# mozack/vdjer

Hardware: AMD Instinct MI355X
Metric: M paired-reads/sec (k-mer build + contig score), IgH 50bp PE (higher is better)
Workload: dtype u8/u64 (2-bit packed bases, integer counts)

## Files before the change

vdjer_amd/csrc/vdjx_kmer.hip:

```cpp
#include "vdjx_common.h"
#include "vdjx_scan.h"
#include "vdjx_part.h"

#include <algorithm>
#include <numeric>
#include <type_traits>
#include <string.h>
#include <stdlib.h>

#define HIST_THREADS 512
#define HIST_BLOCKS 512u
#define LOCAL_SLOTS 2048u
#define K3_SUB_TUPLES g_sub_tuples
__device__ u32 g_sub_tuples = 262144u;
#define NONE32 0xFFFFFFFFu
#define INST_MASK 0x7FFFFFFFu

struct RecView {
	u64 bhi, blo, nm, lq;
};

__device__ inline RecView load_rec(const u64* __restrict__ bases, const u64* __restrict__ nmask,
                                   const u64* __restrict__ lowq, size_t r) {
	RecView v;
// ... 296 lines not shown
                                                    u32 shift, u32 sub_bits, u32* __restrict__ fine_cnt) {
	__shared__ u32 h[PART_MAXB];
	const u32 nbk = 1u << sub_bits;
	for (u32 i = threadIdx.x; i < nbk; i += 512) h[i] = 0;
	__syncthreads();
	size_t t0, t1;
	const u32 seg = part_slice(seg_start, seg_shift, slices, t0, t1);
	for (size_t t = t0 + threadIdx.x; t < t1; t += 512) {
		const TUP x = TUP::load(&in[t]);
		atomicAdd(&h[(u32) (vdjx_bucket_mix(x.lo, x.hi()) >> shift) & (nbk - 1)], 1u);
	}
	__syncthreads();
	for (u32 i = threadIdx.x; i < nbk; i += 512) if (h[i]) atomicAdd(&fine_cnt[((size_t) seg << sub_bits) | i], h[i]);
}

#ifndef RD_THREADS
#define RD_THREADS 768
#define RD_UNR 4
#define RD_WAVES 6
#endif
#define RD_SLOTS 2048u
#define RD_SLOT_BITS 11
#define RD_PQ 4096u
#define RD_LI 512u
#define RD_LROWS 128u
#define RD_MAXLOW 11u
#define ST_CAND 1u
#define ST_MULTI 2u
#define ST_QOK 4u
#define ST_QOK_R 8u
#define ST_ID_SHIFT 8
#define ST_NOID 0xFFFFFFu

struct SurvOutG { u64* lo; u64* hi; u32* gcnt; u64* gfirst; u32* n; u32 cap; u32* n_real; };
#define GC_SHADOW 0x80000000u
#define GC_MASK 0x7FFFFFFFu

__device__ inline bool reads_equal(const u64* __restrict__ bases, const u64* __restrict__ nmask, int rl, u64 a, u64 b) {
	if (rl <= VDJX_SHORT_READ_LEN) {
		const ulonglong2 x = ((const ulonglong2*) bases)[a];
// ... 44 lines not shown
	if (threadIdx.x < 33) cls_cnt[threadIdx.x] = 0;
	__syncthreads();
	for (u32 b = threadIdx.x; b < NB; b += 1024) {
		const u32 n = bucket_start[b + 1] - bucket_start[b];
		atomicAdd(&cls_cnt[n ? 32u - (u32) __builtin_clz(n) : 0u], 1u);
	}
	__syncthreads();
	if (threadIdx.x == 0) { u32 at = 0; for (int cl = 32; cl >= 0; cl--) { cls_at[cl] = at; at += cls_cnt[cl]; } }
	__syncthreads();
	for (u32 b = threadIdx.x; b < NB; b += 1024) {
		const u32 n = bucket_start[b + 1] - bucket_start[b];
		order[atomicAdd(&cls_at[n ? 32u - (u32) __builtin_clz(n) : 0u], 1u)] = b;
	}
}

template <typename TUP, bool SYM = false>
__global__ __launch_bounds__(RD_THREADS, sizeof(TUP) == 16 ? RD_WAVES : RD_WAVES / 2) void k_gated_reduce(const TUP* __restrict__ tup, const u32* __restrict__ bucket_start,
                                                             const u64* __restrict__ bases, const u64* __restrict__ nmask,
                                                             vdjx_qrows quals, int rl, int ob, int k, u64 rec_base,
                                                             u32 mf, u32 cmin, u32 mqq, u32 tlow, SurvOutG so,
                                                             u64* __restrict__ g_distinct, u32* __restrict__ g_err, u32 dbg_in,
                                                             const u32* __restrict__ order) {
#ifdef VDJX_ABLATE
	const u32 dbg = dbg_in;
#else
	const u32 dbg = dbg_in == 9u ? 9u : 0u;
#endif
	typedef typename TUP::hi_t THI;
	__shared__ u64 s_klo[RD_SLOTS];
	__shared__ THI s_khi[RD_SLOTS];
	__shared__ u64 s_first[RD_SLOTS];
	__shared__ u32 s_cnt[RD_SLOTS], s_state[RD_SLOTS];
	__shared__ u32 pq[RD_PQ];
	__shared__ u64 low_inst[RD_LI];
	__shared__ u32 low_n[RD_LROWS];
	__shared__ unsigned short low_slot[RD_LROWS];
	__shared__ u32 s_over, s_ndist, s_nlow, s_npq, s_nsurv, s_base, s_nreal;
	const THI EMPTY = (THI) ~(THI) 0;
	const u32 b = order ? order[blockIdx.x] : blockIdx.x;
	const u32 base = bucket_start[b];
	const u32 n = bucket_start[b + 1] - base;
	const u32 tid = threadIdx.x;
	if (n == 0) return;
	const TUP* T = tup + base;
	const u32 om = (1u << ob) - 1u;
	const u32 per_low = tlow > 1 ? (tlow - 1 < RD_MAXLOW ? tlow - 1 : RD_MAXLOW) : 1;
	const u32 lrows = RD_LI / per_low < RD_LROWS ? RD_LI / per_low : RD_LROWS;
	u32 S = 1;
	while ((u64) S * K3_SUB_TUPLES < n) S <<= 1;
	u32 ndist_total = 0;
	bool verify = S > 1;
	for (;;) {
		if (tid == 0) { s_over = 0; s_ndist = 0; }
		__syncthreads();
		for (u32 s = 0; s < S; s++) {
			for (u32 i = tid; i < RD_SLOTS; i += RD_THREADS) { s_khi[i] = EMPTY; s_cnt[i] = 0; s_first[i] = NONE64; s_state[i] = 0; }
			if (tid == 0) { s_nlow = 0; s_npq = (n >> (32 - RD_SLOT_BITS) || dbg == 9) ? RD_PQ + 1 : 0; s_nsurv = 0; s_nreal = 0; }
			__syncthreads();
			for (u32 t0 = 0; t0 < n; t0 += RD_UNR * RD_THREADS) {
				TUP r_t[RD_UNR];
#pragma unroll
				for (int j = 0; j < RD_UNR; j++) {
					const u32 t = t0 + j * RD_THREADS + tid;
					if (t < n) r_t[j] = TUP::load(&T[t]);
				}
#pragma unroll
				for (int j = 0; j < RD_UNR; j++) {
					const u32 t = t0 + j * RD_THREADS + tid;
					int slot = -1;
					if (t < n) {
						const u32 h = rd_hash(r_t[j].lo, r_t[j].hi());
						if (!(S > 1 && ((h >> 12) & (S - 1)) != s)) {
							slot = lds_insert<THI, RD_SLOTS>(s_klo, s_khi, r_t[j].lo, (THI) r_t[j].hi(), h);
							if (slot < 0) s_over = 1;
						}
					}
					const bool live = slot >= 0 && !verify;
					const u64 inst = r_t[j].inst();
					const u32 c0 = rd_count_min(s_cnt, s_first, (u32) (live ? slot : 0), inst, live);
					bool list = false;
					if (live) {
						u32 st = vdjx_peek(&s_state[slot]);
// ... 2 lines not shown
							if (f != NONE64 && (f >> ob) != (inst >> ob)) {
								const u32 o1 = (u32) inst & om, o0 = (u32) f & om;
								const u32 d = o1 > o0 ? o1 - o0 : o0 - o1;
								if (d && d < (u32) k && !vdjx_kmer_has_period(r_t[j].hi(), r_t[j].lo, k, d)) { atomicOr(&s_state[slot], ST_MULTI); st |= ST_MULTI; }
							}
						}
						list = !((st & ST_MULTI) && c0 + 1 >= tlow);
					}
					const u32 qi = vdjx_wave_inc(&s_npq, list);
					if (list && qi < RD_PQ) pq[qi] = (t << RD_SLOT_BITS) | (u32) slot;
				}
			}
			__syncthreads();
			if (s_over || verify) { if (s_over) break; continue; }
			if (dbg == 1) return;
			for (u32 i = tid; i < RD_SLOTS; i += RD_THREADS) {
				if (s_khi[i] == EMPTY) continue;
				atomicAdd(&s_ndist, SYM ? 2u : 1u);
				const u32 c = s_cnt[i];
				if (c >= cmin) s_state[i] = (s_state[i] & ST_MULTI) | ST_CAND | ((c < tlow ? atomicAdd(&s_nlow, 1u) : ST_NOID) << ST_ID_SHIFT);
			}
			__syncthreads();
			const u32 nlow = s_nlow;
			const bool listed = s_npq <= RD_PQ;
			const u32 nscan = listed ? s_npq : n;
			for (u32 l0 = 0; l0 == 0 || l0 < nlow; l0 += lrows) {
				for (u32 i = tid; i < RD_LROWS; i += RD_THREADS) low_n[i] = 0;
				__syncthreads();
				for (u32 e = tid; e < nscan; e += RD_THREADS) {
					u32 slot, t;
					TUP x;
					if (listed) {
						slot = pq[e] & (RD_SLOTS - 1); t = pq[e] >> RD_SLOT_BITS;
						if (!(vdjx_peek(&s_state[slot]) & ST_CAND)) continue;
						x = TUP::load(&T[t]);
					} else {
						x = TUP::load(&T[e]);
						const u32 h = rd_hash(x.lo, x.hi());
						if (S > 1 && ((h >> 12) & (S - 1)) != s) continue;
						const int sl = lds_lookup<THI, RD_SLOTS>(s_klo, s_khi, x.lo, (THI) x.hi(), h);
						if (sl < 0) continue;
						slot = (u32) sl;
					}
					const u32 st = vdjx_peek(&s_state[slot]);
					if (!(st & ST_CAND)) continue;
					const u64 inst = x.inst(), fi = s_first[slot];
					const u32 lid = st >> ST_ID_SHIFT;
					if (lid != ST_NOID && lid >= l0 && lid < l0 + lrows) {
						const u32 pos = atomicAdd(&low_n[lid - l0], 1u);
						if (pos < per_low) low_inst[(lid - l0) * per_low + pos] = inst;
						low_slot[lid - l0] = (unsigned short) slot;
					}
					if (l0 == 0 && !(st & ST_MULTI) && (inst >> ob) != (fi >> ob)) {
						const u32 o1 = (u32) inst & om, o0 = (u32) fi & om;
						const u32 d = o1 > o0 ? o1 - o0 : o0 - o1;
						if ((d && d < (u32) k && !vdjx_kmer_has_period(x.hi(), x.lo, k, d))
						    || !reads_equal(bases, nmask, rl, (inst >> ob) - rec_base, (fi >> ob) - rec_base)) atomicOr(&s_state[slot], ST_MULTI);
					}
				}
				__syncthreads();
				if (dbg == 4) return;
				const u32 rows = nlow - l0 < lrows ? nlow - l0 : lrows;
				const u32 lane = tid & 63u;
				for (u32 r = tid >> 6; r < (nlow ? rows : 0u); r += RD_THREADS / 64) {
					const u32 slot = low_slot[r], cnt = low_n[r];
					const u64 fi = s_first[slot];
					u32 qv[RD_MAXLOW];
#pragma unroll
					for (u32 i = 0; i < RD_MAXLOW; i++) {
						qv[i] = 33u;
						if (i < cnt && i < per_low) {
							const u64 inst = low_inst[r * per_low + i];
							const uint8_t* q = quals.row((inst >> ob) - rec_base) + (inst == fi ? 0u : (u32) inst & om);
							if (lane < (u32) k) qv[i] = q[lane];
						}
					}
					u32 sum = 0;
#pragma unroll
					for (u32 i = 0; i < RD_MAXLOW; i++) sum += (u32) (uint8_t) (qv[i] - 33u);
					const bool lowq = lane < (u32) k && sum < mqq;
					if (!__ballot(lowq) && lane == 0) atomicOr(&s_state[slot], ST_QOK);
					if (SYM) {
						u64 fr = NONE64;
#pragma unroll
						for (u32 i = 0; i < RD_MAXLOW; i++)
							if (i < cnt && i < per_low) { const u64 m = vdjx_inst_mirror(low_inst[r * per_low + i], ob, rl, k); fr = m < fr ? m : fr; }
#pragma unroll
						for (u32 i = 0; i < RD_MAXLOW; i++) {
							qv[i] = 33u;
							if (i < cnt && i < per_low) {
								const u64 inst = vdjx_inst_mirror(low_inst[r * per_low + i], ob, rl, k);
								const uint8_t* q = quals.row((inst >> ob) - rec_base) + (inst == fr ? 0u : (u32) inst & om);
								if (lane < (u32) k) qv[i] = q[lane];
							}
						}
						u32 sum_r = 0;
#pragma unroll
						for (u32 i = 0; i < RD_MAXLOW; i++) sum_r += (u32) (uint8_t) (qv[i] - 33u);
						const bool lowq_r = lane < (u32) k && sum_r < mqq;
						if (!__ballot(lowq_r) && lane == 0) atomicOr(&s_state[slot], ST_QOK_R);
					}
				}
				__syncthreads();
			}
			if (dbg == 5) return;
			for (u32 i = tid; i < RD_SLOTS; i += RD_THREADS) {
				const u32 st = s_state[i];
				bool keep = false, keep_r = false;
				if (st & ST_CAND) {
					const u32 craw = s_cnt[i];
					const u32 c = craw > 32765u ? 32765u : craw;
					keep = c >= mf && (st & ST_MULTI) && (craw >= tlow || (st & ST_QOK));
					if (SYM) keep_r = c >= mf && (st & ST_MULTI) && (craw >= tlow || (st & ST_QOK_R));
				}
				if (SYM) {
					s_state[i] = (keep || keep_r) ? (atomicAdd(&s_nsurv, 2u) << 2) | (u32) keep | ((u32) keep_r << 1) : NONE32;
					if (keep || keep_r) atomicAdd(&s_nreal, (u32) keep + (u32) keep_r);
				} else s_state[i] = keep ? atomicAdd(&s_nsurv, 1u) : NONE32;
			}
			__syncthreads();
			if (tid == 0) { s_base = s_nsurv ? atomicAdd(so.n, s_nsurv) : 0; if (SYM && s_nreal) atomicAdd(so.n_real, s_nreal); }
			__syncthreads();
			for (u32 i = tid; i < RD_SLOTS; i += RD_THREADS) {
				if (s_state[i] == NONE32) continue;
				u32 pos = s_base + (SYM ? s_state[i] >> 2 : s_state[i]);
				const u32 cgo = s_cnt[i] > 32765u ? 32765u : s_cnt[i];
				if (pos < so.cap) {
					so.lo[pos] = s_klo[i];
					so.hi[pos] = (u64) s_khi[i];
					so.gcnt[pos] = cgo | (SYM && !(s_state[i] & 1u) ? GC_SHADOW : 0u);
					so.gfirst[pos] = s_first[i];
				}
				if (SYM) {
					pos += 1u;
					if (pos < so.cap) {
						u64 rh, rlo;
						vdjx_kmer_rc((u64) s_khi[i], s_klo[i], k, rh, rlo);
						so.lo[pos] = rlo;
// ... 27 lines not shown
static_assert(sizeof(PartialS) == sizeof(Partial), "vdjx_shard_record_bytes(0) is one number");
#define PS_H_BITS 26
#define PS_MAX_SPLIT (1u << (PS_H_BITS - 12))
__device__ inline u64 ps_hi(const PartialS& p) { return p.hic & 0xFFFFFFFFFFFFull; }
__device__ inline u32 ps_cg(const PartialS& p) { const u32 c = (u32) (p.hic >> 48); return (c & 0x7FFFu) | ((c & 0x8000u) ? PART_FLAG : 0u); }
__device__ inline u64 ps_fg(const PartialS& p) { return p.fgh & INST_MASK64; }
__device__ inline u32 ps_h(const PartialS& p) { return (u32) (p.fgh >> INST_BITS); }
#define NEED_SEQ 1u
#define NEED_Q 2u
#define PID_MASK 0x3FFFFFFFu
#define REPLY_KQ 52
#define REPLY_BYTES 408

#define LG_THREADS 768
#define LG_UNR 4
#define LG_FLAG 0x80000000u
#define LG_NOLIST 0x7FFFFFFFu
template <typename TUP, bool SYM = false>
__global__ __launch_bounds__(LG_THREADS, sizeof(TUP) == 16 ? 6 : 3) void k_gated_local(const TUP* __restrict__ tup, const u32* __restrict__ bucket_start,
                                                            const u64* __restrict__ bases, const u64* __restrict__ nmask, u64 rec_base, int k, int rl, int ob,
                                                            u32 tlow, Partial* __restrict__ sparse_g, u32* __restrict__ sparse_ref,
                                                            u32* __restrict__ nd_g, u64* __restrict__ low_inst, u32* __restrict__ g_err,
                                                            const u32* __restrict__ order) {
	typedef typename TUP::hi_t THI;
	const size_t obase = (size_t) bucket_start[order ? order[blockIdx.x] : blockIdx.x];
	__shared__ u64 s_klo[LOCAL_SLOTS];
	__shared__ THI s_khi[LOCAL_SLOTS];
	__shared__ u64 s_mg[LOCAL_SLOTS];
	__shared__ u32 s_cg[LOCAL_SLOTS], s_st[LOCAL_SLOTS];
	__shared__ u32 pq[RD_PQ];
	__shared__ u32 s_ng, s_nlow, s_over, s_npq;
	static_assert(LOCAL_SLOTS == (1u << RD_SLOT_BITS), "list entries carry the slot in RD_SLOT_BITS bits");
	const THI EMPTY = (THI) ~(THI) 0;
	const u32 b = order ? order[blockIdx.x] : blockIdx.x;
	const u32 base = bucket_start[b];
	const u32 n = bucket_start[b + 1] - base;
	const u32 tid = threadIdx.x;
	const u32 om = (1u << ob) - 1u;
	if (n == 0) { if (tid == 0) nd_g[b] = 0; return; }
	const TUP* T = tup + base;
	u32 S = 1;
	while ((u64) S * K3_SUB_TUPLES < n) S <<= 1;
	for (;;) {
		if (tid == 0) { s_ng = 0; s_nlow = 0; s_over = 0; }
		for (u32 s = 0; s < S; s++) {
			for (u32 i = tid; i < LOCAL_SLOTS; i += LG_THREADS) { s_khi[i] = EMPTY; s_cg[i] = 0; s_mg[i] = NONE64; s_st[i] = 0; }
			if (tid == 0) s_npq = n >> (32 - RD_SLOT_BITS) ? RD_PQ + 1 : 0;
			__syncthreads();
			for (u32 t0 = 0; t0 < n; t0 += LG_UNR * LG_THREADS) {
				TUP r_t[LG_UNR];
#pragma unroll
				for (int j = 0; j < LG_UNR; j++) {
					const u32 t = t0 + j * LG_THREADS + tid;
					if (t < n) r_t[j] = TUP::load(&T[t]);
				}
#pragma unroll
				for (int j = 0; j < LG_UNR; j++) {
					const u32 t = t0 + j * LG_THREADS + tid;
					int slot = -1;
					if (t < n) {
						const u32 h = rd_hash(r_t[j].lo, r_t[j].hi());
						if (!(S > 1 && ((h >> 12) & (S - 1)) != s)) {
// ... 6 lines not shown
					const u32 c0 = rd_count_min(s_cg, s_mg, (u32) (live ? slot : 0), inst, live);
					bool list = false;
					if (live) {
						u32 st = vdjx_peek(&s_st[slot]);
						if (!(st & LG_FLAG)) {
							const u64 f = vdjx_peek(&s_mg[slot]);
							if (f != NONE64 && (f >> ob) != (inst >> ob)) {
								const u32 o1 = (u32) inst & om, o0 = (u32) f & om;
								const u32 d = o1 > o0 ? o1 - o0 : o0 - o1;
								if (d && d < (u32) k && !vdjx_kmer_has_period(r_t[j].hi(), r_t[j].lo, k, d)) { atomicOr(&s_st[slot], LG_FLAG); st |= LG_FLAG; }
							}
						}
						list = !((st & LG_FLAG) && c0 + 1 >= tlow);
					}
					const u32 qi = vdjx_wave_inc(&s_npq, list);
					if (list && qi < RD_PQ) pq[qi] = (t << RD_SLOT_BITS) | (u32) slot;
				}
			}
			__syncthreads();
			if (s_over) break;
			for (u32 i = tid; i < LOCAL_SLOTS; i += LG_THREADS) {
				const u32 cg = s_cg[i];
				s_st[i] = (s_st[i] & LG_FLAG) | ((cg && cg < tlow) ? atomicAdd(&s_nlow, cg) : LG_NOLIST);
			}
			__syncthreads();
			const bool listed = s_npq <= RD_PQ;
			const u32 nscan = listed ? s_npq : n;
			for (u32 e = tid; e < nscan; e += LG_THREADS) {
				u32 slot;
				TUP x;
				if (listed) {
					slot = pq[e] & (LOCAL_SLOTS - 1);
					const u32 st0 = vdjx_peek(&s_st[slot]);
					if ((st0 & LG_NOLIST) == LG_NOLIST && (st0 & LG_FLAG)) continue;
					x = TUP::load(&T[pq[e] >> RD_SLOT_BITS]);
				} else {
					x = TUP::load(&T[e]);
					const u32 h = rd_hash(x.lo, x.hi());
					if (S > 1 && ((h >> 12) & (S - 1)) != s) continue;
					const int sl = lds_lookup<THI, LOCAL_SLOTS>(s_klo, s_khi, x.lo, (THI) x.hi(), h);
					if (sl < 0) continue;
					slot = (u32) sl;
				}
				const u32 st = vdjx_peek(&s_st[slot]);
				const u32 loff = st & LG_NOLIST;
				const u64 inst = x.inst();
				u32 cg = vdjx_peek(&s_cg[slot]);
				if (loff != LG_NOLIST) {
					cg &= 0xFFFFu;
					low_inst[base + loff + (atomicAdd(&s_cg[slot], 0x10000u) >> 16)] = inst;
// ... 1188 lines not shown

inline u32 ceil_log2_u64(u64 x) { u32 b = 0; while ((1ull << b) < x) b++; return b; }

static bool sync_debug() { static const bool on = vdjx_env_set("VDJX_SYNC_DEBUG"); return on; }
static void dbg_sync(vdjx_ctx* c, const char* what) {
	if (!sync_debug()) return;
	const hipError_t e = hipStreamSynchronize(c->stream);
	fprintf(stderr, "[vdjx] %s: %s\n", what, hipGetErrorString(e));
}

struct GatedHist { u32 HB = 0, NBH = 0, N = 0; u32* hstart = nullptr; bool sym = false; };
static bool build_sym(const vdjx_pool* pool, int k) {
	return pool->sym && pool->W == 2 && (k & 1) && pool->n_records % 2 == 0;
}
static bool sym_walk_wanted() { static const bool on = !vdjx_env_set("VDJX_NO_SYM_WALK"); return on; }
static size_t gated_bucket_default() { static const size_t v = (size_t) vdjx_env_num("VDJX_GATED_BUCKET", 3072, 1, 1ll << 32); return v; }
template <typename A>
int stage_gated_hist(vdjx_ctx* c, A& db, const vdjx_pool* pool, int k, size_t per_bucket, u64 geometry_instances, GatedHist* gh, bool sym = false) {
	hipStream_t st = c->stream;
	const size_t R = sym ? pool->n_records / 2 : pool->n_records;
	const int P = pool->rl - k + 1;
	const u64 NI = geometry_instances ? geometry_instances : (u64) R * (u64) P;
	const size_t per = per_bucket ? per_bucket : gated_bucket_default();
	const u32 hb_max = pool->W > 2 ? 14u : 15u;
	u32 HB = ceil_log2_u64((NI + per - 1) / per);
	HB = std::max(8u, std::min(hb_max, HB));
	const u32 NBH = 1u << HB;
#ifdef VDJX_ABLATE
	static const u32 hist_dbg = (u32) vdjx_env_num("VDJX_HIST_DBG", 0, 0, 4);
#else
	constexpr u32 hist_dbg = 0;
#endif
	u32 nblk = (u32) std::min<size_t>(HIST_BLOCKS, (R + 4095) / 4096);
	if (nblk == 0) nblk = 1;
	size_t rpb = (R + nblk - 1) / nblk;
	u32 *hcnt, *hstart;
	HIP_TRY(db.alloc(&hcnt, NBH));
	HIP_TRY(db.alloc(&hstart, NBH + 1));
// ... 12 lines not shown
	dbg_sync(c, "k_gated_hist");
	vdjx_scan_one(st, hcnt, NBH, hstart);
	HIP_TRY(hipMemcpyAsync(c->h_pin, hstart + NBH, 4, hipMemcpyDeviceToHost, st));
	HIP_TRY(hipStreamSynchronize(st));
	HIP_TRY(hipGetLastError());
#ifdef VDJX_ABLATE
	if (hist_dbg) return VDJX_ESTATE;
#endif
	const u32 N = *(const u32*) c->h_pin;
	c->stats["gated_instances"] = sym ? 2ull * N : N;
	gh->HB = HB; gh->NBH = NBH; gh->N = N; gh->hstart = hstart; gh->sym = sym;
	return VDJX_OK;
}

template <typename TUP, typename A>
int stage_gated_cut(vdjx_ctx* c, A& db, const vdjx_pool* pool, u64 rec_base, int k, size_t per_bucket, u64 geometry_instances, const GatedHist& gh, GTuples<TUP>* out) {
	hipStream_t st = c->stream;
	const bool sym = gh.sym;
	const size_t R = sym ? pool->n_records / 2 : pool->n_records;
	const int P = pool->rl - k + 1;
	const size_t per = per_bucket ? per_bucket : gated_bucket_default();
	const u32 hb_max = pool->W > 2 ? 14u : 15u;
	const bool lng = pool->W > 2;
	const u32 HB = gh.HB, NBH = gh.NBH, N = gh.N;
	u32* hstart = gh.hstart;
	size_t rpb;
	out->N = N;
	const u64 Ng = geometry_instances ? geometry_instances : (u64) N;
	static const size_t refine = (size_t) vdjx_env_num("VDJX_REFINE_TUPLES", 4096, 1, 1ll << 32);
	u32 T = 8;
	while (T < HB && ((u64) per << T) < Ng) T++;
	u32 extra = 0;
	const size_t refine_at = per_bucket ? std::max<size_t>(per_bucket, refine / 2) : refine;
	if (T == HB && HB == hb_max && Ng / NBH > refine_at) {
		extra = 1;
		while (extra < 5 && (Ng >> extra) / NBH > refine_at) extra++;
	}
	const u32 Tt = T + extra;
	const u32 NBt = 1u << Tt;
	HIP_TRY(db.alloc(&out->t, (size_t) N + 1));
	constexpr u32 stage_tuples = PARTR_STAGE_BYTES / (u32) sizeof(TUP);
	constexpr u32 lds_partr = PARTR_STAGE_BYTES + stage_tuples * 4;
	u32 cbits = Tt, fbits = 0;
	if (Tt > 10) { cbits = extra ? Tt - 10 : 8; fbits = Tt - cbits; }
// ... 29 lines not shown
		vdjx_scan_one(st, fine_cnt, NBt, tstart);
	} else {
		hipLaunchKernelGGL(k_pick_u32, dim3((NBt + 1 + 255) / 256), dim3(256), 0, st, hstart, 1u << (HB - Tt), NBt + 1, tstart);
	}
	if (fbits) {
		u32* gcur2;
		HIP_TRY(db.alloc(&gcur2, NBt));
		vdjx_prof_scope ps(c, "k_part_tuples");
		HIP_TRY(part_launch(st, k_part<TUP, TupBucket<TUP>, part_segs>, NBc * slices, PART_LDS_BYTES, tstart, NBt, 0u, gcur2, out->t,
		                    l1, part_segs{hstart, HB - cbits, slices, fbits}, TupBucket<TUP>{64 - Tt, (1u << fbits) - 1u}));
	}
	return VDJX_OK;
}

template <typename TUP, typename A>
int stage_gated_partition(vdjx_ctx* c, A& db, const vdjx_pool* pool, u64 rec_base, int k, size_t per_bucket, u64 geometry_instances, GTuples<TUP>* out, bool sym = false) {
	GatedHist gh;
	int rc = stage_gated_hist(c, db, pool, k, per_bucket, geometry_instances, &gh, sym);
	if (rc) return rc;
	return stage_gated_cut<TUP>(c, db, pool, rec_base, k, per_bucket, geometry_instances, gh, out);
}

static int set_sub_tuples(vdjx_ctx* c) {
	static const u32 sub = (u32) vdjx_env_num("VDJX_SUB_TUPLES", 262144, 1, 0xFFFFFFFFll);
	if (c->sub_tuples_set != sub) {
		HIP_TRY(hipMemcpyToSymbolAsync(HIP_SYMBOL(g_sub_tuples), &sub, 4, 0, hipMemcpyHostToDevice, c->stream));
		c->sub_tuples_set = sub;
	}
	return VDJX_OK;
}
template <typename TUP, typename A>
int bucket_order(vdjx_ctx* c, A& db, const GTuples<TUP>& t, u32** order) {
	*order = nullptr;
	if (t.NB < 1024) return VDJX_OK;
	HIP_TRY(db.alloc(order, t.NB));
// ... 14 lines not shown
	const u32 cap = (sym ? t.N : t.N / 2) + 16;
	u32 *g_err, *n_surv;
	u64* g_distinct;
	HIP_TRY(db.alloc(&sv->lo, cap)); HIP_TRY(db.alloc(&sv->hi, cap)); HIP_TRY(db.alloc(&sv->gcnt, cap)); HIP_TRY(db.alloc(&sv->gfirst, cap));
	HIP_TRY(db.alloc(&g_distinct, 64 * 16 + 2));
	g_err = (u32*) (g_distinct + 64 * 16);
	n_surv = g_err + 1;
	u32* n_real = g_err + 2;
	HIP_TRY(hipMemsetAsync(g_distinct, 0, (64 * 16 + 2) * 8, st));
	SurvOutG so{sv->lo, sv->hi, sv->gcnt, sv->gfirst, n_surv, cap, n_real};
	static const u32 rd_dbg = (u32) vdjx_env_num("VDJX_RD_DBG", 0, 0, 9);
	if (t.N) {
		vdjx_prof_scope ps(c, "k_gated_reduce");
		u32* order;
		if ((rc = bucket_order(c, db, t, &order))) return rc;
		if (sym) hipLaunchKernelGGL((k_gated_reduce<TUP, true>), dim3(t.NB), dim3(RD_THREADS), 0, st, t.t, t.bucket_start, pv.bases, pv.nmask, pv.quals, pv.rl, pv.ob, k, rec_base,
		                            mfu, cmin, mqq, tlow, so, g_distinct, g_err, rd_dbg, (const u32*) order);
		else hipLaunchKernelGGL(k_gated_reduce<TUP>, dim3(t.NB), dim3(RD_THREADS), 0, st, t.t, t.bucket_start, pv.bases, pv.nmask, pv.quals, pv.rl, pv.ob, k, rec_base,
		                        mfu, cmin, mqq, tlow, so, g_distinct, g_err, rd_dbg, (const u32*) order);
	}
	u64* spread = (u64*) c->h_pin;
	u32* tail = (u32*) (spread + 64 * 16);
	static_assert((64 * 16 + 2) * 8 == VDJX_HPIN_SYNC_BYTES, "h_pin layout (vdjx_common.h)");
	HIP_TRY(hipMemcpyAsync(spread, g_distinct, VDJX_HPIN_SYNC_BYTES, hipMemcpyDeviceToHost, st));
	HIP_TRY(hipStreamSynchronize(st));
	HIP_TRY(hipGetLastError());
	const u32 ns = tail[1], err = tail[0];
	if (err) { vdjx_set_error("k_gated_reduce: %u buckets could not be split to fit LDS", err); return VDJX_EHIP; }
	if (ns > cap) { vdjx_set_error("survivor capacity logic failed (%u > %u)", ns, cap); return VDJX_EHIP; }
	sv->ndist = 0;
// ... 380 lines not shown
	HIP_TRY(hipStreamSynchronize(st));
	HIP_TRY(hipGetLastError());
	n_roots = *(const u32*) c->h_pin;
	g->n_roots = n_roots;
	vdjx_prof_collect(c, false);
	return VDJX_OK;
}

template <typename TUP>
int kmer_build_impl2(vdjx_ctx* c, const vdjx_pool* pool, int k, int mf, int mq, vdjx_graph* g) {
	const int P = pool->rl - k + 1;
	vdjx_work db(c);
	GTuples<TUP> t;
	const bool sym = build_sym(pool, k);
	c->stats["kmer_build_sym"] = sym ? 1 : 0;
	int rc = stage_gated_partition<TUP>(c, db, pool, 0, k, 0, 0, &t, sym);
	if (rc) return rc;
	PoolView pv{pool->d_bases, pool->d_nmask, vdjx_qrows{pool->d_quals, pool->d_quals2, pool->q_split, pool->qstride}, pool->rl, pool->ob};
	SurvivorsG sv;
	rc = stage_gated_reduce<TUP>(c, db, t, pv, 0, k, mf, mq, &sv, sym);
	if (rc) return rc;
	vdjx_ri_open_gate(c);
	dbg_sync(c, "gated_reduce");
	g->pre_nodes = (size_t) sv.ndist;
	RecountOut ro{};
	if (sv.n) {
		HIP_TRY(db.alloc(&sv.ucnt, sv.n)); HIP_TRY(db.alloc(&sv.ufirst, sv.n));
		HIP_TRY(db.alloc(&ro.in_first, (size_t) sv.n * 4)); HIP_TRY(db.alloc(&ro.in_from, (size_t) sv.n * 4));
		HIP_TRY(db.alloc(&ro.edge_first, (size_t) sv.n * 4)); HIP_TRY(db.alloc(&ro.edge_to, (size_t) sv.n * 4));
		ro.ucnt = sv.ucnt; ro.ufirst = sv.ufirst;
		for (int attempt = 0; attempt < 2; attempt++) {
// ... 136 lines not shown
static u64 shard_geometry_bound(const vdjx_shard* s) {
	const int P = s->pool->rl - s->k + 1;
	return std::max<u64>(1, s->rec_stride * (u64) P / 4);
}

template <typename TUP>
static int shard_local_impl(vdjx_shard* s) {
	vdjx_ctx* c = s->c;
	hipStream_t st = c->stream;
	PersistAlloc db(c);
	const u64 rec_base = s->rec_base();
	GTuples<TUP> t;
	int rc = VDJX_OK;
	if (s->have_hist && s->gh.sym != s->sym) s->have_hist = false;
	const size_t per_b = 0;
	if (!s->have_hist) rc = stage_gated_hist(c, db, s->pool, s->k, per_b, shard_geometry_bound(s) / (s->sym ? 2 : 1), &s->gh, s->sym);
	if (rc) return rc;
	s->have_hist = true;
	const size_t cap = (size_t) s->gh.N + 1;
	const size_t nb_max = ((size_t) 1 << 20) + 16 * (size_t) s->nranks + 2;
	Partial* sparse;
	u32 *g_err, *sparse_ref;
	HIP_TRY(db.alloc(&s->low_inst, cap));
	HIP_TRY(db.alloc(&s->dense_ref, cap));
	HIP_TRY(db.alloc(&s->nd, nb_max));
	HIP_TRY(db.alloc(&s->dstart, nb_max + 1));
	HIP_TRY(db.alloc(&g_err, 1));
	u32* keep_starts;
	HIP_TRY(db.alloc(&keep_starts, nb_max + 1));
	s->fill_mark = db.mark();
	HIP_TRY(db.alloc(&sparse, cap));
	HIP_TRY(db.alloc(&sparse_ref, cap));
	const vdjx_arena::mark_t tuple_mark = db.mark();
	rc = stage_gated_cut<TUP>(c, db, s->pool, rec_base, s->k, per_b, (s->agreed ? s->agreed : shard_geometry_bound(s)) / (s->sym ? 2 : 1), s->gh, &t);
	if (rc) return rc;
	if (t.NB < (u32) s->nranks) { vdjx_set_error("vdjx_shard_local: fewer buckets (%u) than ranks", t.NB); return VDJX_ELIMIT; }
	s->NBo = t.NB / (u32) s->nranks;
	if (s->NBo * (u32) s->nranks != t.NB) s->NBo = (s->NBo + 1 + 15) & ~15u;
	s->NBf = s->NBo * (u32) s->nranks;
	if ((size_t) s->NBf + 1 > nb_max) { vdjx_set_error("vdjx_shard_local: %u buckets", s->NBf); return VDJX_ELIMIT; }
	HIP_TRY(hipMemsetAsync(g_err, 0, 4, st));
	if (s->NBf > t.NB) HIP_TRY(hipMemsetAsync(s->nd + t.NB, 0, (size_t) (s->NBf - t.NB) * 4, st));
	if ((rc = set_sub_tuples(c))) return rc;
	{
		vdjx_prof_scope ps(c, "k_gated_local");
		u32* order;
		if ((rc = bucket_order(c, db, t, &order))) return rc;
		if (s->sym) hipLaunchKernelGGL((k_gated_local<TUP, true>), dim3(t.NB), dim3(LG_THREADS), 0, st, t.t, t.bucket_start, s->pool->d_bases, s->pool->d_nmask, rec_base,
		                               s->k, s->pool->rl, s->pool->ob, s->tlow, sparse, sparse_ref, s->nd, s->low_inst, g_err, (const u32*) order);
// ... 54 lines not shown
	if (s->sparse) {
		PersistAlloc db(s->c);
		db.release_to(s->fill_mark);
		s->sparse = nullptr; s->sparse_ref = nullptr; s->tuple_bucket_start = nullptr;
	}
	return VDJX_OK;
}

extern "C" int vdjx_shard_count(vdjx_shard* s, uint64_t* gated_instances) {
	if (!s || !gated_instances) { vdjx_set_error("vdjx_shard_count: NULL argument"); return VDJX_EINVAL; }
	if (s->phase != 0) { vdjx_set_error("vdjx_shard_count: call it before vdjx_shard_local"); return VDJX_ESTATE; }
	HIP_TRY(hipSetDevice(s->c->device));
	vdjx_clear_errors();
	if (!s->have_hist) {
		PersistAlloc db(s->c);
		const int rc = stage_gated_hist(s->c, db, s->pool, s->k, 0, shard_geometry_bound(s) / (s->sym_capable ? 2 : 1), &s->gh, s->sym_capable);
		if (rc) return rc;
		s->have_hist = true;
	}
	*gated_instances = (u64) s->gh.N * (s->gh.sym ? 2 : 1);
	return VDJX_OK;
}
extern "C" int vdjx_shard_symmetric(const vdjx_shard* s) { return s && s->sym_capable ? 1 : 0; }
extern "C" int vdjx_shard_geometry2(vdjx_shard* s, uint64_t agreed_instances, int all_symmetric) {
	if (!s) { vdjx_set_error("vdjx_shard_geometry2: NULL argument"); return VDJX_EINVAL; }
	if (all_symmetric && !s->sym_capable) { vdjx_set_error("vdjx_shard_geometry2: this rank's pool is not made of couples"); return VDJX_EINVAL; }
	const int rc = vdjx_shard_geometry(s, agreed_instances);
	if (rc) return rc;
	s->sym = all_symmetric != 0;
	s->c->stats["kmer_build_sym"] = s->sym ? 1 : 0;
	return VDJX_OK;
// ... 433 lines not shown
```

Baseline: 918.8.

## Template gated-reduce geometry; prefetch first tuple batch; hoist read-compare loads

Geometry constants for the gated reduce kernel (threads, slot bits, pq size, low rows, bucket size) become a template traits struct, with a narrower variant available for 16-byte tuples. The default stays wide, and bucket and refine sizes are now derived from that geometry. The first batch of tuples is loaded before the hash table clear so global load latency overlaps the LDS init. The read-equality loads are issued before the low-row atomics, and the symmetric mirror-quality pass is merged into the forward loop. The extra registers for hoisted loads and merged SYM arrays could lower occupancy.

Result: no change. 919.7 (median of 2 runs) (+0.1%).

```diff
diff --git a/vdjer_amd/csrc/vdjx_kmer.hip b/vdjer_amd/csrc/vdjx_kmer.hip
--- a/vdjer_amd/csrc/vdjx_kmer.hip
+++ b/vdjer_amd/csrc/vdjx_kmer.hip
@@ -334,16 +334,13 @@
 	for (u32 i = threadIdx.x; i < nbk; i += 512) if (h[i]) atomicAdd(&fine_cnt[((size_t) seg << sub_bits) | i], h[i]);
 }
 
-#ifndef RD_THREADS
-#define RD_THREADS 768
-#define RD_UNR 4
-#define RD_WAVES 6
+struct RdWide   { static constexpr u32 THREADS = 768, UNR = 4, WAVES = 6, SLOT_BITS = 11, PQ = 4096, LI = 512, LROWS = 128, BUCKET = 3072; };
+struct RdNarrow { static constexpr u32 THREADS = 384, UNR = 4, WAVES = 6, SLOT_BITS = 10, PQ = 2048, LI = 256, LROWS = 64, BUCKET = 1536; };
+#ifndef VDJX_RD_GEOM16
+#define VDJX_RD_GEOM16 RdWide
 #endif
-#define RD_SLOTS 2048u
-#define RD_SLOT_BITS 11
-#define RD_PQ 4096u
-#define RD_LI 512u
-#define RD_LROWS 128u
+template <typename TUP> struct RdGeomOf { typedef RdWide type; };
+template <> struct RdGeomOf<Tup16> { typedef VDJX_RD_GEOM16 type; };
 #define RD_MAXLOW 11u
 #define ST_CAND 1u
 #define ST_MULTI 2u
@@ -418,8 +415,10 @@
 	}
 }
 
-template <typename TUP, bool SYM = false>
-__global__ __launch_bounds__(RD_THREADS, sizeof(TUP) == 16 ? RD_WAVES : RD_WAVES / 2) void k_gated_reduce(const TUP* __restrict__ tup, const u32* __restrict__ bucket_start,
+__device__ inline u32 rd_again(u32 x) { asm volatile("" : "+v"(x)); return x; }
+
+template <typename TUP, bool SYM = false, typename G = typename RdGeomOf<TUP>::type>
+__global__ __launch_bounds__(G::THREADS, sizeof(TUP) == 16 ? G::WAVES : G::WAVES / 2) void k_gated_reduce(const TUP* __restrict__ tup, const u32* __restrict__ bucket_start,
                                                              const u64* __restrict__ bases, const u64* __restrict__ nmask,
                                                              vdjx_qrows quals, int rl, int ob, int k, u64 rec_base,
                                                              u32 mf, u32 cmin, u32 mqq, u32 tlow, SurvOutG so,
@@ -431,6 +430,9 @@
 	const u32 dbg = dbg_in == 9u ? 9u : 0u;
 #endif
 	typedef typename TUP::hi_t THI;
+	constexpr u32 RD_THREADS = G::THREADS, RD_UNR = G::UNR, RD_SLOT_BITS = G::SLOT_BITS, RD_SLOTS = 1u << G::SLOT_BITS, RD_PQ = G::PQ, RD_LI = G::LI, RD_LROWS = G::LROWS;
+	static_assert(RD_SLOT_BITS <= 16, "low_slot is 16 bits wide");
+	static_assert(RD_LI >= RD_MAXLOW, "a round holds at least one row of the longest kind");
 	__shared__ u64 s_klo[RD_SLOTS];
 	__shared__ THI s_khi[RD_SLOTS];
 	__shared__ u64 s_first[RD_SLOTS];
@@ -458,18 +460,26 @@
 		if (tid == 0) { s_over = 0; s_ndist = 0; }
 		__syncthreads();
 		for (u32 s = 0; s < S; s++) {
-			for (u32 i = tid; i < RD_SLOTS; i += RD_THREADS) { s_khi[i] = EMPTY; s_cnt[i] = 0; s_first[i] = NONE64; s_state[i] = 0; }
-			if (tid == 0) { s_nlow = 0; s_npq = (n >> (32 - RD_SLOT_BITS) || dbg == 9) ? RD_PQ + 1 : 0; s_nsurv = 0; s_nreal = 0; }
+			TUP r_t[RD_UNR];
+			const u32 tid0 = rd_again(tid);
+#pragma unroll
+			for (u32 j = 0; j < RD_UNR; j++) {
+				const u32 t = j * RD_THREADS + tid0;
+				if (t < n) r_t[j] = TUP::load(&T[t]);
+			}
+			for (u32 i = rd_again(tid); i < RD_SLOTS; i += RD_THREADS) { s_khi[i] = EMPTY; s_cnt[i] = 0; s_first[i] = NONE64; s_state[i] = 0; }
+			if (tid == 0) { s_nlow = 0; s_npq = (rd_again(n) >> (32 - RD_SLOT_BITS) || dbg == 9) ? RD_PQ + 1 : 0; s_nsurv = 0; s_nreal = 0; }
 			__syncthreads();
 			for (u32 t0 = 0; t0 < n; t0 += RD_UNR * RD_THREADS) {
-				TUP r_t[RD_UNR];
+				if (t0) {
 #pragma unroll
-				for (int j = 0; j < RD_UNR; j++) {
-					const u32 t = t0 + j * RD_THREADS + tid;
-					if (t < n) r_t[j] = TUP::load(&T[t]);
+					for (u32 j = 0; j < RD_UNR; j++) {
+						const u32 t = t0 + j * RD_THREADS + tid;
+						if (t < n) r_t[j] = TUP::load(&T[t]);
+					}
 				}
 #pragma unroll
-				for (int j = 0; j < RD_UNR; j++) {
+				for (u32 j = 0; j < RD_UNR; j++) {
 					const u32 t = t0 + j * RD_THREADS + tid;
 					int slot = -1;
 					if (t < n) {
@@ -502,7 +512,7 @@
 			__syncthreads();
 			if (s_over || verify) { if (s_over) break; continue; }
 			if (dbg == 1) return;
-			for (u32 i = tid; i < RD_SLOTS; i += RD_THREADS) {
+			for (u32 i = rd_again(tid); i < RD_SLOTS; i += RD_THREADS) {
 				if (s_khi[i] == EMPTY) continue;
 				atomicAdd(&s_ndist, SYM ? 2u : 1u);
 				const u32 c = s_cnt[i];
@@ -513,15 +523,16 @@
 			const bool listed = s_npq <= RD_PQ;
 			const u32 nscan = listed ? s_npq : n;
 			for (u32 l0 = 0; l0 == 0 || l0 < nlow; l0 += lrows) {
-				for (u32 i = tid; i < RD_LROWS; i += RD_THREADS) low_n[i] = 0;
+				for (u32 i = rd_again(tid); i < RD_LROWS; i += RD_THREADS) low_n[i] = 0;
 				__syncthreads();
-				for (u32 e = tid; e < nscan; e += RD_THREADS) {
-					u32 slot, t;
+				for (u32 e = rd_again(tid); e < nscan; e += RD_THREADS) {
+					u32 slot = 0;
 					TUP x;
 					if (listed) {
-						slot = pq[e] & (RD_SLOTS - 1); t = pq[e] >> RD_SLOT_BITS;
+						const u32 ent = pq[e];
+						slot = ent & (RD_SLOTS - 1);
 						if (!(vdjx_peek(&s_state[slot]) & ST_CAND)) continue;
-						x = TUP::load(&T[t]);
+						x = TUP::load(&T[ent >> RD_SLOT_BITS]);
 					} else {
 						x = TUP::load(&T[e]);
 						const u32 h = rd_hash(x.lo, x.hi());
@@ -533,58 +544,68 @@
 					const u32 st = vdjx_peek(&s_state[slot]);
 					if (!(st & ST_CAND)) continue;
 					const u64 inst = x.inst(), fi = s_first[slot];
+					bool cmp = false;
+					ulonglong2 ra = make_ulonglong2(0, 0), rb = ra;
+					u64 na = 0, nb = 0;
+					const bool early = rl <= VDJX_SHORT_READ_LEN;
+					if (l0 == 0 && !(st & ST_MULTI) && (inst >> ob) != (fi >> ob)) {
+						const u32 o1 = (u32) inst & om, o0 = (u32) fi & om;
+						const u32 d = o1 > o0 ? o1 - o0 : o0 - o1;
+						if (d && d < (u32) k && !vdjx_kmer_has_period(x.hi(), x.lo, k, d)) atomicOr(&s_state[slot], ST_MULTI);
+						else {
+							cmp = true;
+							if (early) {
+								const u64 a = (inst >> ob) - rec_base, b2 = (fi >> ob) - rec_base;
+								ra = ((const ulonglong2*) bases)[a]; rb = ((const ulonglong2*) bases)[b2];
+								na = nmask[a]; nb = nmask[b2];
+							}
+						}
+					}
 					const u32 lid = st >> ST_ID_SHIFT;
 					if (lid != ST_NOID && lid >= l0 && lid < l0 + lrows) {
 						const u32 pos = atomicAdd(&low_n[lid - l0], 1u);
 						if (pos < per_low) low_inst[(lid - l0) * per_low + pos] = inst;
 						low_slot[lid - l0] = (unsigned short) slot;
 					}
-					if (l0 == 0 && !(st & ST_MULTI) && (inst >> ob) != (fi >> ob)) {
-						const u32 o1 = (u32) inst & om, o0 = (u32) fi & om;
-						const u32 d = o1 > o0 ? o1 - o0 : o0 - o1;
-						if ((d && d < (u32) k && !vdjx_kmer_has_period(x.hi(), x.lo, k, d))
-						    || !reads_equal(bases, nmask, rl, (inst >> ob) - rec_base, (fi >> ob) - rec_base)) atomicOr(&s_state[slot], ST_MULTI);
+					if (cmp) {
+						const bool eq = early ? (ra.x == rb.x && ra.y == rb.y && na == nb)
+						                      : reads_equal(bases, nmask, rl, (inst >> ob) - rec_base, (fi >> ob) - rec_base);
+						if (!eq) atomicOr(&s_state[slot], ST_MULTI);
 					}
 				}
 				__syncthreads();
 				if (dbg == 4) return;
 				const u32 rows = nlow - l0 < lrows ? nlow - l0 : lrows;
-				const u32 lane = tid & 63u;
-				for (u32 r = tid >> 6; r < (nlow ? rows : 0u); r += RD_THREADS / 64) {
-					const u32 slot = low_slot[r], cnt = low_n[r];
+				const u32 lane = __lane_id();
+				for (u32 r = rd_again(tid) >> 6; r < (nlow ? rows : 0u); r += RD_THREADS / 64) {
+					const u32 slot = low_slot[r], cnt = low_n[r] < per_low ? low_n[r] : per_low;
 					const u64 fi = s_first[slot];
-					u32 qv[RD_MAXLOW];
+					u64 fr = NONE64;
+					if (SYM) {
+#pragma unroll
+						for (u32 i = 0; i < RD_MAXLOW; i++)
+							if (i < cnt) { const u64 m = vdjx_inst_mirror(low_inst[r * per_low + i], ob, rl, k); fr = m < fr ? m : fr; }
+					}
+					u32 qv[RD_MAXLOW], qr[SYM ? RD_MAXLOW : 1u];
 #pragma unroll
 					for (u32 i = 0; i < RD_MAXLOW; i++) {
 						qv[i] = 33u;
-						if (i < cnt && i < per_low) {
+						if (SYM) qr[i] = 33u;
+						if (i < cnt && lane < (u32) k) {
 							const u64 inst = low_inst[r * per_low + i];
-							const uint8_t* q = quals.row((inst >> ob) - rec_base) + (inst == fi ? 0u : (u32) inst & om);
-							if (lane < (u32) k) qv[i] = q[lane];
+							qv[i] = (quals.row((inst >> ob) - rec_base) + (inst == fi ? 0u : (u32) inst & om))[lane];
+							if (SYM) {
+								const u64 m = vdjx_inst_mirror(inst, ob, rl, k);
+								qr[i] = (quals.row((m >> ob) - rec_base) + (m == fr ? 0u : (u32) m & om))[lane];
+							}
 						}
 					}
-					u32 sum = 0;
+					u32 sum = 0, sum_r = 0;
 #pragma unroll
-					for (u32 i = 0; i < RD_MAXLOW; i++) sum += (u32) (uint8_t) (qv[i] - 33u);
+					for (u32 i = 0; i < RD_MAXLOW; i++) { sum += (u32) (uint8_t) (qv[i] - 33u); if (SYM) sum_r += (u32) (uint8_t) (qr[i] - 33u); }
 					const bool lowq = lane < (u32) k && sum < mqq;
 					if (!__ballot(lowq) && lane == 0) atomicOr(&s_state[slot], ST_QOK);
 					if (SYM) {
-						u64 fr = NONE64;
-#pragma unroll
-						for (u32 i = 0; i < RD_MAXLOW; i++)
-							if (i < cnt && i < per_low) { const u64 m = vdjx_inst_mirror(low_inst[r * per_low + i], ob, rl, k); fr = m < fr ? m : fr; }
-#pragma unroll
-						for (u32 i = 0; i < RD_MAXLOW; i++) {
-							qv[i] = 33u;
-							if (i < cnt && i < per_low) {
-								const u64 inst = vdjx_inst_mirror(low_inst[r * per_low + i], ob, rl, k);
-								const uint8_t* q = quals.row((inst >> ob) - rec_base) + (inst == fr ? 0u : (u32) inst & om);
-								if (lane < (u32) k) qv[i] = q[lane];
-							}
-						}
-						u32 sum_r = 0;
-#pragma unroll
-						for (u32 i = 0; i < RD_MAXLOW; i++) sum_r += (u32) (uint8_t) (qv[i] - 33u);
 						const bool lowq_r = lane < (u32) k && sum_r < mqq;
 						if (!__ballot(lowq_r) && lane == 0) atomicOr(&s_state[slot], ST_QOK_R);
 					}
@@ -592,7 +613,7 @@
 				__syncthreads();
 			}
 			if (dbg == 5) return;
-			for (u32 i = tid; i < RD_SLOTS; i += RD_THREADS) {
+			for (u32 i = rd_again(tid); i < RD_SLOTS; i += RD_THREADS) {
 				const u32 st = s_state[i];
 				bool keep = false, keep_r = false;
 				if (st & ST_CAND) {
@@ -609,7 +630,7 @@
 			__syncthreads();
 			if (tid == 0) { s_base = s_nsurv ? atomicAdd(so.n, s_nsurv) : 0; if (SYM && s_nreal) atomicAdd(so.n_real, s_nreal); }
 			__syncthreads();
-			for (u32 i = tid; i < RD_SLOTS; i += RD_THREADS) {
+			for (u32 i = rd_again(tid); i < RD_SLOTS; i += RD_THREADS) {
 				if (s_state[i] == NONE32) continue;
 				u32 pos = s_base + (SYM ? s_state[i] >> 2 : s_state[i]);
 				const u32 cgo = s_cnt[i] > 32765u ? 32765u : s_cnt[i];
@@ -667,6 +688,9 @@
 
 #define LG_THREADS 768
 #define LG_UNR 4
+#define LG_BUCKET 3072u
+#define LG_PQ 4096u
+#define LG_SLOT_BITS 11
 #define LG_FLAG 0x80000000u
 #define LG_NOLIST 0x7FFFFFFFu
 template <typename TUP, bool SYM = false>
@@ -681,9 +705,9 @@
 	__shared__ THI s_khi[LOCAL_SLOTS];
 	__shared__ u64 s_mg[LOCAL_SLOTS];
 	__shared__ u32 s_cg[LOCAL_SLOTS], s_st[LOCAL_SLOTS];
-	__shared__ u32 pq[RD_PQ];
+	__shared__ u32 pq[LG_PQ];
 	__shared__ u32 s_ng, s_nlow, s_over, s_npq;
-	static_assert(LOCAL_SLOTS == (1u << RD_SLOT_BITS), "list entries carry the slot in RD_SLOT_BITS bits");
+	static_assert(LOCAL_SLOTS == (1u << LG_SLOT_BITS), "list entries carry the slot in LG_SLOT_BITS bits");
 	const THI EMPTY = (THI) ~(THI) 0;
 	const u32 b = order ? order[blockIdx.x] : blockIdx.x;
 	const u32 base = bucket_start[b];
@@ -698,7 +722,7 @@
 		if (tid == 0) { s_ng = 0; s_nlow = 0; s_over = 0; }
 		for (u32 s = 0; s < S; s++) {
 			for (u32 i = tid; i < LOCAL_SLOTS; i += LG_THREADS) { s_khi[i] = EMPTY; s_cg[i] = 0; s_mg[i] = NONE64; s_st[i] = 0; }
-			if (tid == 0) s_npq = n >> (32 - RD_SLOT_BITS) ? RD_PQ + 1 : 0;
+			if (tid == 0) s_npq = n >> (32 - LG_SLOT_BITS) ? LG_PQ + 1 : 0;
 			__syncthreads();
 			for (u32 t0 = 0; t0 < n; t0 += LG_UNR * LG_THREADS) {
 				TUP r_t[LG_UNR];
@@ -735,7 +759,7 @@
 						list = !((st & LG_FLAG) && c0 + 1 >= tlow);
 					}
 					const u32 qi = vdjx_wave_inc(&s_npq, list);
-					if (list && qi < RD_PQ) pq[qi] = (t << RD_SLOT_BITS) | (u32) slot;
+					if (list && qi < LG_PQ) pq[qi] = (t << LG_SLOT_BITS) | (u32) slot;
 				}
 			}
 			__syncthreads();
@@ -745,7 +769,7 @@
 				s_st[i] = (s_st[i] & LG_FLAG) | ((cg && cg < tlow) ? atomicAdd(&s_nlow, cg) : LG_NOLIST);
 			}
 			__syncthreads();
-			const bool listed = s_npq <= RD_PQ;
+			const bool listed = s_npq <= LG_PQ;
 			const u32 nscan = listed ? s_npq : n;
 			for (u32 e = tid; e < nscan; e += LG_THREADS) {
 				u32 slot;
@@ -754,7 +778,7 @@
 					slot = pq[e] & (LOCAL_SLOTS - 1);
 					const u32 st0 = vdjx_peek(&s_st[slot]);
 					if ((st0 & LG_NOLIST) == LG_NOLIST && (st0 & LG_FLAG)) continue;
-					x = TUP::load(&T[pq[e] >> RD_SLOT_BITS]);
+					x = TUP::load(&T[pq[e] >> LG_SLOT_BITS]);
 				} else {
 					x = TUP::load(&T[e]);
 					const u32 h = rd_hash(x.lo, x.hi());
@@ -1973,14 +1997,14 @@
 	return pool->sym && pool->W == 2 && (k & 1) && pool->n_records % 2 == 0;
 }
 static bool sym_walk_wanted() { static const bool on = !vdjx_env_set("VDJX_NO_SYM_WALK"); return on; }
-static size_t gated_bucket_default() { static const size_t v = (size_t) vdjx_env_num("VDJX_GATED_BUCKET", 3072, 1, 1ll << 32); return v; }
+static size_t gated_bucket_default(size_t geom) { static const size_t v = (size_t) vdjx_env_num("VDJX_GATED_BUCKET", 0, 1, 1ll << 32); return v ? v : geom; }
 template <typename A>
-int stage_gated_hist(vdjx_ctx* c, A& db, const vdjx_pool* pool, int k, size_t per_bucket, u64 geometry_instances, GatedHist* gh, bool sym = false) {
+int stage_gated_hist(vdjx_ctx* c, A& db, const vdjx_pool* pool, int k, size_t per_bucket, size_t geom_bucket, u64 geometry_instances, GatedHist* gh, bool sym = false) {
 	hipStream_t st = c->stream;
 	const size_t R = sym ? pool->n_records / 2 : pool->n_records;
 	const int P = pool->rl - k + 1;
 	const u64 NI = geometry_instances ? geometry_instances : (u64) R * (u64) P;
-	const size_t per = per_bucket ? per_bucket : gated_bucket_default();
+	const size_t per = per_bucket ? per_bucket : gated_bucket_default(geom_bucket);
 	const u32 hb_max = pool->W > 2 ? 14u : 15u;
 	u32 HB = ceil_log2_u64((NI + per - 1) / per);
 	HB = std::max(8u, std::min(hb_max, HB));
@@ -2023,12 +2047,12 @@
 }
 
 template <typename TUP, typename A>
-int stage_gated_cut(vdjx_ctx* c, A& db, const vdjx_pool* pool, u64 rec_base, int k, size_t per_bucket, u64 geometry_instances, const GatedHist& gh, GTuples<TUP>* out) {
+int stage_gated_cut(vdjx_ctx* c, A& db, const vdjx_pool* pool, u64 rec_base, int k, size_t per_bucket, size_t geom_bucket, u64 geometry_instances, const GatedHist& gh, GTuples<TUP>* out) {
 	hipStream_t st = c->stream;
 	const bool sym = gh.sym;
 	const size_t R = sym ? pool->n_records / 2 : pool->n_records;
 	const int P = pool->rl - k + 1;
-	const size_t per = per_bucket ? per_bucket : gated_bucket_default();
+	const size_t per = per_bucket ? per_bucket : gated_bucket_default(geom_bucket);
 	const u32 hb_max = pool->W > 2 ? 14u : 15u;
 	const bool lng = pool->W > 2;
 	const u32 HB = gh.HB, NBH = gh.NBH, N = gh.N;
@@ -2036,7 +2060,8 @@
 	size_t rpb;
 	out->N = N;
 	const u64 Ng = geometry_instances ? geometry_instances : (u64) N;
-	static const size_t refine = (size_t) vdjx_env_num("VDJX_REFINE_TUPLES", 4096, 1, 1ll << 32);
+	static const size_t refine_env = (size_t) vdjx_env_num("VDJX_REFINE_TUPLES", 0, 1, 1ll << 32);
+	const size_t refine = refine_env ? refine_env : geom_bucket * 4 / 3;
 	u32 T = 8;
 	while (T < HB && ((u64) per << T) < Ng) T++;
 	u32 extra = 0;
@@ -2096,11 +2121,11 @@
 }
 
 template <typename TUP, typename A>
-int stage_gated_partition(vdjx_ctx* c, A& db, const vdjx_pool* pool, u64 rec_base, int k, size_t per_bucket, u64 geometry_instances, GTuples<TUP>* out, bool sym = false) {
+int stage_gated_partition(vdjx_ctx* c, A& db, const vdjx_pool* pool, u64 rec_base, int k, size_t per_bucket, size_t geom_bucket, u64 geometry_instances, GTuples<TUP>* out, bool sym = false) {
 	GatedHist gh;
-	int rc = stage_gated_hist(c, db, pool, k, per_bucket, geometry_instances, &gh, sym);
+	int rc = stage_gated_hist(c, db, pool, k, per_bucket, geom_bucket, geometry_instances, &gh, sym);
 	if (rc) return rc;
-	return stage_gated_cut<TUP>(c, db, pool, rec_base, k, per_bucket, geometry_instances, gh, out);
+	return stage_gated_cut<TUP>(c, db, pool, rec_base, k, per_bucket, geom_bucket, geometry_instances, gh, out);
 }
 
 static int set_sub_tuples(vdjx_ctx* c) {
@@ -2145,6 +2170,7 @@
 		vdjx_prof_scope ps(c, "k_gated_reduce");
 		u32* order;
 		if ((rc = bucket_order(c, db, t, &order))) return rc;
+		constexpr u32 RD_THREADS = RdGeomOf<TUP>::type::THREADS;
 		if (sym) hipLaunchKernelGGL((k_gated_reduce<TUP, true>), dim3(t.NB), dim3(RD_THREADS), 0, st, t.t, t.bucket_start, pv.bases, pv.nmask, pv.quals, pv.rl, pv.ob, k, rec_base,
 		                            mfu, cmin, mqq, tlow, so, g_distinct, g_err, rd_dbg, (const u32*) order);
 		else hipLaunchKernelGGL(k_gated_reduce<TUP>, dim3(t.NB), dim3(RD_THREADS), 0, st, t.t, t.bucket_start, pv.bases, pv.nmask, pv.quals, pv.rl, pv.ob, k, rec_base,
@@ -2555,7 +2581,7 @@
 	GTuples<TUP> t;
 	const bool sym = build_sym(pool, k);
 	c->stats["kmer_build_sym"] = sym ? 1 : 0;
-	int rc = stage_gated_partition<TUP>(c, db, pool, 0, k, 0, 0, &t, sym);
+	int rc = stage_gated_partition<TUP>(c, db, pool, 0, k, 0, RdGeomOf<TUP>::type::BUCKET, 0, &t, sym);
 	if (rc) return rc;
 	PoolView pv{pool->d_bases, pool->d_nmask, vdjx_qrows{pool->d_quals, pool->d_quals2, pool->q_split, pool->qstride}, pool->rl, pool->ob};
 	SurvivorsG sv;
@@ -2722,7 +2748,7 @@
 	int rc = VDJX_OK;
 	if (s->have_hist && s->gh.sym != s->sym) s->have_hist = false;
 	const size_t per_b = 0;
-	if (!s->have_hist) rc = stage_gated_hist(c, db, s->pool, s->k, per_b, shard_geometry_bound(s) / (s->sym ? 2 : 1), &s->gh, s->sym);
+	if (!s->have_hist) rc = stage_gated_hist(c, db, s->pool, s->k, per_b, LG_BUCKET, shard_geometry_bound(s) / (s->sym ? 2 : 1), &s->gh, s->sym);
 	if (rc) return rc;
 	s->have_hist = true;
 	const size_t cap = (size_t) s->gh.N + 1;
@@ -2740,7 +2766,7 @@
 	HIP_TRY(db.alloc(&sparse, cap));
 	HIP_TRY(db.alloc(&sparse_ref, cap));
 	const vdjx_arena::mark_t tuple_mark = db.mark();
-	rc = stage_gated_cut<TUP>(c, db, s->pool, rec_base, s->k, per_b, (s->agreed ? s->agreed : shard_geometry_bound(s)) / (s->sym ? 2 : 1), s->gh, &t);
+	rc = stage_gated_cut<TUP>(c, db, s->pool, rec_base, s->k, per_b, LG_BUCKET, (s->agreed ? s->agreed : shard_geometry_bound(s)) / (s->sym ? 2 : 1), s->gh, &t);
 	if (rc) return rc;
 	if (t.NB < (u32) s->nranks) { vdjx_set_error("vdjx_shard_local: fewer buckets (%u) than ranks", t.NB); return VDJX_ELIMIT; }
 	s->NBo = t.NB / (u32) s->nranks;
@@ -2825,7 +2851,7 @@
 	vdjx_clear_errors();
 	if (!s->have_hist) {
 		PersistAlloc db(s->c);
-		const int rc = stage_gated_hist(s->c, db, s->pool, s->k, 0, shard_geometry_bound(s) / (s->sym_capable ? 2 : 1), &s->gh, s->sym_capable);
+		const int rc = stage_gated_hist(s->c, db, s->pool, s->k, 0, LG_BUCKET, shard_geometry_bound(s) / (s->sym_capable ? 2 : 1), &s->gh, s->sym_capable);
 		if (rc) return rc;
 		s->have_hist = true;
 	}
```
